# dwkim606/optimal_conv

Measured on AMD Instinct MI355X. Metric: homomorphic convs/sec (conv_then_pack + BN bias, k x k, batch B, N=2^16), higher is better.
Workload: dtype u64; 1 GPU; conv 3 3; ker_wid=3, batch=256, in_wid=16, logN=16, moduli=ckks.DefaultBootstrapParams[6] Q0,Q1 + P=0x1fffffffffe00001, ciphertexts_per_launch_set=4, contexts_per_gpu=4, chunk_nodes=512

## Files before the change

### optimal_conv_amd/csrc/hc_kernels.h

```cpp
#pragma once
#include "hc_arith.h"

#define HC_TPB 256
#ifndef HC_MIN_WAVES
#define HC_MIN_WAVES 4
#endif
#define HC_ROWS_LDS 4096
#define HC_COLS_LDS 4096

struct __attribute__((aligned(16))) HcTw { u64 w, ws; };

#define HC_SMALL_Q(q) ((q) < (1ull << 31))
template <bool B> struct HcBool { static constexpr bool value = B; };
template <int V> struct HcInt { static constexpr int value = V; };
#define HC_COUNT_DISPATCH(n, body) do { switch (n) { case 1: body(HcInt<1>{}); break; case 2: body(HcInt<2>{}); break; case 3: body(HcInt<3>{}); break; case 4: body(HcInt<4>{}); break; \
    case 5: body(HcInt<5>{}); break; case 6: body(HcInt<6>{}); break; case 7: body(HcInt<7>{}); break; case 8: body(HcInt<8>{}); break; default: break; } } while (0)
#define HC_LD(S32, rowptr, j) ((S32) ? hc_ld32(rowptr, j) : (rowptr)[j])
#define HC_ST(S32, rowptr, j, v) do { if (S32) hc_st32(rowptr, j, v); else (rowptr)[j] = (v); } while (0)
#define HC_ROW_DISPATCH(row32, body) do { if (row32) body(HcBool<true>{}); else body(HcBool<false>{}); } while (0)
__device__ __forceinline__ u64 hc_ld32(const u64 *row, size_t j) { return (u64)reinterpret_cast<const u32 *>(row)[j]; }
__device__ __forceinline__ void hc_st32(u64 *row, size_t j, u64 v) { reinterpret_cast<u32 *>(row)[j] = (u32)v; }
struct __attribute__((packed, aligned(4))) HcU64A4 { u64 v; };
__device__ __forceinline__ u64 hc_ldp(const u64 *row, size_t j, bool row32) {
    return reinterpret_cast<const HcU64A4 *>(reinterpret_cast<const char *>(row) + (j << (row32 ? 2 : 3)))->v & (row32 ? 0xFFFFFFFFull : ~0ull);
// ... 1287 lines not shown
                lds[a0] = hc_submod(hc_addmod(hc_submod(Y0[j], m0, q), g0, q), hc_canon8(e0[kk], Q), q);
            }
        }
        __syncthreads();
#pragma unroll
        for (int j = 0; j < HC_B5_ROWS; j++) {
            const int kk = b + j;
            const u32 srcidx = hc_perm_src((u32)((HC_TILE * 16 + kk) * 256 + t), B.gal);
            const u64 d1 = lds[hc_rows_lds(kk ^ 8, (int)(srcidx & 255))], d0 = lds[hc_rows_lds(kk, (int)(srcidx & 255))];
            o[65536 + kk * 256] = FM == HC_FM_FREE ? hc_reduce64(s1[j] + d1, B.m0.mu, Q) : hc_addmod(s1[j], d1, q);
            o[kk * 256] = FM == HC_FM_FREE ? hc_reduce64(s0[j] + d0, B.m0.mu, Q) : hc_addmod(s0[j], d0, q);
        }
    }
}

#define HC_STPB 256
#define HC_STILES 64
#define HC_S_LDS 1024
__device__ __forceinline__ int hc_s_addr(int line, int x) { return x * 4 + line; }
__device__ __forceinline__ int hc_s_pos(int u, int lo) { return (u & ((1 << lo) - 1)) | ((u >> lo) << (lo + 2)); }
template <bool ROWS, int D> __device__ __forceinline__ HcTw hc_s_tw_fwd(const HcTwTab &T, int x, int gline) {
    if (D >= 16) { constexpr int s = D == 128 ? 0 : D == 64 ? 1 : D == 32 ? 2 : 3; const int slot = (1 << s) - 1 + (x >> (8 - s)); return ROWS ? T.rowsA[gline * 16 + slot] : T.colsA[slot]; }
    constexpr int s = D == 8 ? 0 : D == 4 ? 1 : D == 2 ? 2 : 3; const int slot = (1 << s) - 1 + ((x & 15) >> (4 - s));
    return ROWS ? T.rowsB[gline * 256 + slot * 16 + (x >> 4)] : T.colsB[slot * 16 + (x >> 4)];
}
template <bool ROWS, int D> __device__ __forceinline__ HcTw hc_s_tw_inv(const HcTwTab &T, int x, int gline) {
    if (D <= 8) { constexpr int s = D == 1 ? 0 : D == 2 ? 1 : D == 4 ? 2 : 3; const int slot = (8 >> s) - 1 + ((x & 15) >> (s + 1)); return ROWS ? T.rowsB[gline * 256 + slot * 16 + (x >> 4)] : T.colsB[slot * 16 + (x >> 4)]; }
    constexpr int s = D == 16 ? 0 : D == 32 ? 1 : D == 64 ? 2 : 3; const int slot = (8 >> s) - 1 + (x >> (5 + s));
    return ROWS ? T.rowsA[gline * 16 + slot] : T.colsA[slot];
}
// ... 1495 lines not shown
```

### optimal_conv_amd/csrc/hconv.hip

```cpp
#ifdef HC_EMU
#include "hip_emu.h"
#else
#include <hip/hip_runtime.h>
#endif

#include <math.h>
#include <stdarg.h>
#include <stdio.h>
#include <string.h>

#include <map>
#include <utility>
#include <string>
#include <vector>

#include "../../include/hconv.h"
#include "../../include/hconv_test_hooks.h"
#include "hc_kernels.h"
#include "hc_gomath.h"
#ifndef HC_GX_LV
#define HC_GX_LV 64
#endif
#ifndef HC_GX_PW
#define HC_GX_PW 32
#endif
// ... 62 lines not shown
    HcTwTab32 fwd32 = {nullptr, nullptr, nullptr, nullptr}, inv32 = {nullptr, nullptr, nullptr, nullptr};
    HcTwTab inv_f64;
    std::vector<void *> allocs;
};
struct HcEvk { HcTw *q_rows; HcTw *p_rows; u64 *q_mont; bool row_local; bool row256; };
struct HcSwk { u64 *rows = nullptr; int level = 0, beta = 0; };
struct HcProfRec { std::string name; hipEvent_t a, b; };
struct hc_ctx {
    int device = 0, nq = 0, np = 0;
    hipStream_t stream = nullptr;
    std::vector<HcModHost> mods;
    std::map<u64, HcEvk> evk;
    std::map<u64, HcSwk> swk;
    HcTw *idx_pairs = nullptr;
    u64 *idx_mont = nullptr;
    u64 *ws_cts = nullptr; size_t ws_cts_rows = 0;
    u64 *ws_cts2 = nullptr; size_t ws_cts2_rows = 0;
    HcTw *ws_ctc = nullptr; size_t ws_ctc_cts = 0;
    u64 *ws_tmp = nullptr; size_t ws_tmp_rows = 0;
    HcMod *d_mods = nullptr; HcTw *d_csts = nullptr;
    u64 *d_mono = nullptr;
    struct CacheBlk { size_t n = 0; hipEvent_t ev = nullptr; bool pending = false; };
    std::map<char *, CacheBlk> cache_blk; std::map<size_t, std::vector<void *>> cache_free;
    int async_alloc = 0;
#ifdef HC_EMU
    long small_mm_wgs = 0;
#else
    long small_mm_wgs = 1024;
#endif
    long allocs_live = 0;
// ... 15 lines not shown
    u64 *ws_gather = nullptr; size_t ws_gather_rows = 0;
    long small_levels = 16;
    long peer_access = 1;
    int xcd_rows = 1;
    int pack32 = 1;
    int rot_fuse = 1;
    int small32 = 1;
    unsigned peer_warned = 0;
    unsigned peer_enabled = 0;
    long profile = 0;
    std::vector<HcProfRec> prof;
    std::map<std::string, std::pair<double, long>> prof_acc;
    hipEvent_t t0 = nullptr, t1 = nullptr;
    std::string err;
};
struct hc_ker { u64 *d = nullptr; int max_ob = 0; };

static std::string g_create_err;
static int hc_fail(hc_ctx *c, int code, const char *fmt, ...) {
    char buf[512]; va_list ap; va_start(ap, fmt); vsnprintf(buf, sizeof buf, fmt, ap); va_end(ap);
    if (c) c->err = buf; else g_create_err = buf;
    return code;
}
#define HC_HIP(c, call) do { hipError_t e_ = (call); if (e_ != hipSuccess) return hc_fail(c, HC_ERR_HIP, "%s: %s", #call, hipGetErrorString(e_)); } while (0)
#define HC_ENTER(c) do { if (!(c)) return HC_ERR_ARG; HC_HIP(c, hipSetDevice((c)->device)); } while (0)
static void hc_hoist_drop(hc_ctx *c) { c->hoist_cx = nullptr; }
static void hc_hoist_hold(hc_ctx *c, const void *cx, int level) { c->hoist_cx = cx; c->hoist_level = level; }
static int hc_hoist_need(hc_ctx *c, const char *fn, const void *cx, int level) {
    if (c->hoist_cx == cx && c->hoist_level == level) return HC_OK;
    return hc_fail(c, HC_ERR_STATE, "%s: no decomposition of this polynomial at level %d is held (call hc_keyswitch_decompose first)", fn, level);
}
// ... 580 lines not shown
    A->ctc = c->ws_ctc; A->ker = kers; A->tmp = c->ws_tmp; A->cts = cts; A->i0 = 0; A->norm = norm; A->slot0 = 0; A->slot_step = norm;
    A->cts_stride = cts_stride;
    A->m0 = m0.m; A->m1 = m1.m;
    A->q1inv = h_pair(h_inv(m1.m.q % m0.m.q, m0.m.q), m0.m.q);
    A->h = (m1.m.q - 1) >> 1; A->negh0 = m0.m.q - (A->h % m0.m.q);
    return HC_OK;
}

static int hc_prepare_ctc(hc_ctx *c, const HcPtrs &ct_in, int n, const u64 cst[2]) {
    HC_TRY(hc_ensure_ctc(c, (size_t)n));
    HcCtc K; K.m0 = c->mods[0].m; K.m1 = c->mods[1].m;
    K.c0 = h_pair(cst[0] % K.m0.q, K.m0.q); K.c1 = h_pair(cst[1] % K.m1.q, K.m1.q);
    return hc_launch(c, "ctc", hc_k_ctc_pairs, dim3(64, 4, (unsigned)n), ct_in, c->ws_ctc, K);
}

static int hc_loopA_run_set(hc_ctx *c, const HcPtrs &kers, int n, int i_first, int i_stride, int nch, u64 *cts, size_t cts_stride, bool compact, int gm = 1) {
    long chunk = (c->chunk_nodes < 1 ? 1 : c->chunk_nodes) / n; if (chunk < 1) chunk = 1;
    if (chunk > nch) chunk = nch;
    HC_TRY(hc_ensure_tmp(c, (size_t)n * (size_t)chunk * 2));
    HcLoopA A; HC_TRY(hc_fill_loopA(c, &A, kers, cts, cts_stride, i_stride));
    const HcModHost &m0 = c->mods[0], &m1 = c->mods[1];
    for (int j0 = 0; j0 < nch; j0 += (int)chunk) {
        const int nj = (int)((nch - j0) < chunk ? (nch - j0) : chunk);
        A.i0 = i_first + j0 * i_stride;
        A.slot0 = compact ? j0 : A.i0; A.slot_step = compact ? 1 : i_stride;
        A.njobs = 2 * nj; A.gm = gm;
        const dim3 pair = hc_grid(nj, n), flat = hc_grid(2 * nj * n);
        if (gm > 1) {
            const bool f64 = hc_f64_ok(m1.m.q);
            const HcTwTab &t1 = f64 ? m1.inv_f64 : m1.inv;
            HC_TRY(f64 ? hc_launch(c, "a1g_mulsum_rowsinv", hc_k_a1g<1>, pair, A, t1) : hc_launch(c, "a1g_mulsum_rowsinv", hc_k_a1g<0>, pair, A, t1));
            if (f64) HC_TRY(hc_fm_free(m0.m.q) ? hc_launch(c, "a2_colsinv_lift_colsfwd", hc_k_a2<HC_FM_FREE, 1>, flat, A, t1, m0.fwd) : hc_launch(c, "a2_colsinv_lift_colsfwd", hc_k_a2<HC_FM_ALT, 1>, flat, A, t1, m0.fwd));
            else HC_TRY(hc_fm_free(m0.m.q) ? hc_launch(c, "a2_colsinv_lift_colsfwd", hc_k_a2<HC_FM_FREE, 0>, flat, A, t1, m0.fwd) : hc_launch(c, "a2_colsinv_lift_colsfwd", hc_k_a2<HC_FM_ALT, 0>, flat, A, t1, m0.fwd));
            HC_TRY(HC_LAUNCH_FM(m0.m.q, c, "a3g_rowsfwd_sum_rescale", hc_k_a3g, pair, A, m0.fwd));
            continue;
        }
        if (hc_f64_ok(m1.m.q)) {
            HC_TRY(hc_launch(c, "a1_mul_rowsinv", hc_k_a1p<1>, pair, A, m1.inv_f64));
            HC_TRY(hc_fm_free(m0.m.q) ? hc_launch(c, "a2_colsinv_lift_colsfwd", hc_k_a2<HC_FM_FREE, 1>, flat, A, m1.inv_f64, m0.fwd)
                                      : hc_launch(c, "a2_colsinv_lift_colsfwd", hc_k_a2<HC_FM_ALT, 1>, flat, A, m1.inv_f64, m0.fwd));
// ... 95 lines not shown
    if (!rc) rc = hc_launch(c, "evk_div_p", hc_k_pointwise<HC_PW_MULC>, hc_pw_grid(2 * HC_N), (const u64 *)stageq, (const u64 *)stageq, stageq, (size_t)2 * HC_N, m0.m, pinv);
    if (!rc) rc = hc_launch(c, "make_pairs", hc_k_make_pairs, hc_pw_grid(2 * HC_N), (const u64 *)stageq, e.q_rows, (size_t)2 * HC_N, m0.m.q, 0);
    if (!rc) rc = hc_launch(c, "evk_to_mont", hc_k_pointwise<HC_PW_TO_MONT>, hc_pw_grid(2 * HC_N), (const u64 *)stageq, (const u64 *)stageq, e.q_mont, (size_t)2 * HC_N, m0.m, z);
    if (!rc) rc = hc_launch(c, "evk_from_mont", hc_k_pointwise<HC_PW_FROM_MONT>, hc_pw_grid(2 * HC_N), (const u64 *)stage, (const u64 *)stage, stage, (size_t)2 * HC_N, mp.m, z);
    if (!rc) rc = hc_launch(c, "evk_ninv", hc_k_pointwise<HC_PW_MULC>, hc_pw_grid(2 * HC_N), (const u64 *)stage, (const u64 *)stage, stage, (size_t)2 * HC_N, mp.m, h_pair(mp.m.ninv, mp.m.q));
    if (!rc) rc = hc_launch(c, "make_pairs", hc_k_make_pairs, hc_pw_grid(2 * HC_N), (const u64 *)stage, e.p_rows, (size_t)2 * HC_N, mp.m.q, 1);
    if (hipStreamSynchronize(c->stream) != hipSuccess && !rc) rc = hc_fail(c, HC_ERR_HIP, "hc_evk_load: stream synchronize failed");
    if (rc) return rc;
    S.keep(e.q_rows); S.keep(e.p_rows);
    auto it = c->evk.find(galEl);
    if (it != c->evk.end()) { hcx_free(c, it->second.q_rows); hcx_free(c, it->second.p_rows); }
    c->evk[galEl] = e;
    return HC_OK;
}

extern "C" int hc_idx_load(hc_ctx *c, const uint64_t *idx_host) {
    HC_ENTER(c);
    const HcModHost &m0 = c->mods[0];
    HcScratch S(c);
    u64 *stage = nullptr; HC_HIP(c, S.alloc(&stage, (size_t)HC_LOGN * HC_N * sizeof(u64)));
    if (idx_host) {
        HC_HIP(c, hcx_h2d_async(c, stage, idx_host, (size_t)HC_LOGN * HC_N * sizeof(u64)));
    } else {
        HC_HIP(c, hipMemsetAsync(stage, 0, (size_t)HC_LOGN * HC_N * sizeof(u64), c->stream));
        u64 one = 1;
        for (int i = 0; i < HC_LOGN; i++) HC_HIP(c, hcx_h2d_async(c, stage + (size_t)i * HC_N + ((size_t)1 << i), &one, sizeof one));
        HC_HIP(c, hipStreamSynchronize(c->stream));
        u64 *tmp = nullptr; HC_HIP(c, S.alloc(&tmp, (size_t)HC_LOGN * HC_N * sizeof(u64)));
        HC_TRY(HC_LAUNCH_FM(m0.m.q, c, "cols_fwd", hc_k_cols_fwd, dim3(16, HC_LOGN), (const u64 *)stage, tmp, m0.fwd, m0.m.q));
        HC_TRY(HC_LAUNCH_FM(m0.m.q, c, "rows_fwd_canon", hc_k_rows_fwd_canon, dim3(16, HC_LOGN), (const u64 *)tmp, stage, m0.fwd, m0.m.q, m0.m.mu));
    }
    HcTw *pairs = nullptr; HC_HIP(c, S.alloc(&pairs, (size_t)HC_LOGN * HC_N * (sizeof(HcTw) + sizeof(u64))));
    u64 *mont = reinterpret_cast<u64 *>(pairs + (size_t)HC_LOGN * HC_N);
    HcTw z; z.w = z.ws = 0;
    HC_TRY(hc_launch(c, "idx_pairs", hc_k_make_pairs, hc_pw_grid((size_t)HC_LOGN * HC_N), (const u64 *)stage, pairs, (size_t)HC_LOGN * HC_N, m0.m.q, 0));
    HC_TRY(hc_launch(c, "idx_to_mont", hc_k_pointwise<HC_PW_TO_MONT>, hc_pw_grid((size_t)HC_LOGN * HC_N), (const u64 *)stage, (const u64 *)stage, mont, (size_t)HC_LOGN * HC_N, m0.m, z));
    HC_HIP(c, hipStreamSynchronize(c->stream));
    S.keep(pairs);
    if (c->idx_pairs) HC_HIP(c, hcx_free(c, c->idx_pairs));
    c->idx_pairs = pairs; c->idx_mont = mont;
    return HC_OK;
}

static int hc_ker_from_device(hc_ctx *c, u64 *d, int max_ob, bool take, hc_ker **out) {
    u64 *dst = d;
    int rc = HC_OK;
    if (!take) {
        HC_HIP(c, hcx_malloc(c, (void **)&dst, (size_t)max_ob * 2 * HC_N * sizeof(u64)));
        if (hipMemcpyAsync(dst, d, (size_t)max_ob * 2 * HC_N * sizeof(u64), hipMemcpyDeviceToDevice, c->stream) != hipSuccess) rc = hc_fail(c, HC_ERR_HIP, "hc_ker_load: device copy failed");
    }
    if (!rc && hipStreamSynchronize(c->stream) != hipSuccess) rc = hc_fail(c, HC_ERR_HIP, "hc_ker_load: stream synchronize failed");
    if (rc) { hcx_free(c, dst); return rc; }
    hc_ker *k = new hc_ker(); k->d = dst; k->max_ob = max_ob; *out = k;
    return HC_OK;
}
// ... 58 lines not shown
                              int real_ib, int real_ob, int norm, double scale, int trans, hc_ker **out) {
    HC_ENTER(c);
    return hc_prep_ker_impl(c, trans ? "hc_prep_ker_ex" : "hc_prep_ker", ker_in, ker_len, bn_a, in_wid, ker_wid, real_ib, real_ob, norm, scale, trans, 1, 1, out);
}
extern "C" int hc_prep_ker(hc_ctx *c, const double *ker_in, int ker_len, const double *bn_a, int in_wid, int ker_wid,
                           int real_ib, int real_ob, int norm, double scale, hc_ker **out) {
    return hc_prep_ker_ex(c, ker_in, ker_len, bn_a, in_wid, ker_wid, real_ib, real_ob, norm, scale, 0, out);
}
extern "C" int hc_ker_download(hc_ctx *c, const hc_ker *k, uint64_t *host_out) {
    HC_ENTER(c); if (!k || !host_out) return hc_fail(c, HC_ERR_ARG, "hc_ker_download: null");
    const size_t n = (size_t)k->max_ob * 2 * HC_N;
    HC_HIP(c, hipMemcpyAsync(host_out, k->d, n * sizeof(u64), hipMemcpyDeviceToHost, c->stream));
    HC_HIP(c, hipStreamSynchronize(c->stream));
    return HC_OK;
}
extern "C" void hc_ker_free(hc_ctx *c, hc_ker *k) { if (!k) return; if (c) { hipSetDevice(c->device); hipStreamSynchronize(c->stream); } hcx_free(c, k->d); delete k; }

static int hc_fill_loopB(hc_ctx *c, HcLoopB *B, const u64 *src, u64 *dst, const HcEvk &e, int logStep, int step, int norm, u64 galEl, int chunk) {
    const HcModHost &m0 = c->mods[0], &mp = c->mods[(size_t)c->nq];
    B->src = src; B->dst = dst;
    B->tmpC = c->ws_tmp; B->tmpE = c->ws_tmp + (size_t)chunk * HC_N; B->tmpT = c->ws_tmp + (size_t)chunk * 3 * HC_N;
    B->idx = c->idx_pairs + (size_t)logStep * HC_N;
    B->evkQ = e.q_rows; B->evkP = e.p_rows;
    B->idxM = c->idx_mont + (size_t)logStep * HC_N; B->evkQM = e.q_mont;
    B->n0 = 0; B->step = step; B->norm = norm; B->nodes = 1; B->src_stride = 0; B->dst_stride = 0;
    B->m0 = m0.m; B->mp = mp.m;
    B->pmodq = h_pair(mp.m.q % m0.m.q, m0.m.q);
    B->pinv = h_pair(h_inv(mp.m.q % m0.m.q, m0.m.q), m0.m.q);
    B->mu0 = (u64)((((u128)1) << 64) / m0.m.q);
    {
        const double pf = (double)mp.m.q;
        u64 lo = 0, hi = mp.m.q;
        while (lo < hi) { u64 mid = lo + (hi - lo) / 2; if ((u64)((double)mid / pf) >= 1) hi = mid; else lo = mid + 1; }
        B->vthresh = lo;
    }
    B->gal = (u32)(galEl & 0x1FFFF);
    return HC_OK;
}
static int hc_pack_level(hc_ctx *c, const u64 *src, u64 *dst, size_t sstride, size_t dstride, int n, int step, int logStep, int norm, u64 galEl, const HcPtrs *bias_last, const HcPtrs *outs_last = nullptr) {
    auto it = c->evk.find(galEl);
    if (it == c->evk.end()) return hc_fail(c, HC_ERR_STATE, "pack: no switching key loaded for galEl=%llu (the reference panics in permuteNTT)", (unsigned long long)galEl);
    if (!it->second.row_local) return hc_fail(c, HC_ERR_UNSUPPORTED, "pack: galEl=%llu does not permute inside 4096-coefficient tiles (needs max_cnum <= 4096)", (unsigned long long)galEl);
    if (!c->idx_pairs) HC_TRY(hc_idx_load(c, nullptr));
    const int nodes = (step + norm - 1) / norm;
    long chunkl = (c->chunk_nodes < 1 ? 1 : c->chunk_nodes) / n; if (chunkl < 1) chunkl = 1;
    const int chunk = (int)(chunkl < nodes ? chunkl : nodes);
    HC_TRY(hc_ensure_tmp(c, (size_t)n * chunk * 4));
    HcLoopB B; HC_TRY(hc_fill_loopB(c, &B, src, dst, it->second, logStep, step, norm, galEl, n * chunk));
    B.src_stride = sstride; B.dst_stride = dstride;
    if (it->second.row256) B.tmpT = nullptr;
    HcPtrs nobias; memset(&nobias, 0, sizeof nobias);
    const HcModHost &m0 = c->mods[0], &mp = c->mods[(size_t)c->nq];
    for (int n0 = 0; n0 < nodes; n0 += chunk) {
        const int nn = (nodes - n0) < chunk ? (nodes - n0) : chunk;
        B.n0 = n0; B.nodes = nn;
        const dim3 g1 = hc_grid(n * nn), g2 = hc_grid(2 * n * nn);
        if (c->small_levels > 0 && (long)n * nn <= c->small_levels && it->second.row256) {
            const HcPtrs pb = bias_last ? *bias_last : nobias, po = outs_last ? *outs_last : nobias;
            B.tmpT = nullptr;
            const dim3 s1(HC_STILES, (unsigned)(n * nn)), s2(HC_STILES, (unsigned)(2 * n * nn)), s3(HC_STILES, (unsigned)(n * nn), 2);
            HC_TRY(hc_launch<HC_STPB>(c, "b1_node_rowsinv", hc_k_sb1, s1, B, m0.inv));
            HC_TRY(hc_launch<HC_STPB>(c, "b2_colsinv_colsfwdP", hc_k_sb2, s1, B, m0.inv, mp.fwd));
            HC_TRY(hc_launch<HC_STPB>(c, "b3_rowsfwdP_mac_rowsinvP", hc_k_sb3, s3, B, mp.fwd, mp.inv));
            HC_TRY(hc_launch<HC_STPB>(c, "b4_colsinvP_modup_colsfwd", hc_k_sb4, s2, B, mp.inv, m0.fwd));
            HC_TRY(hc_launch<HC_STPB>(c, "b5_rowsfwd_moddown_perm_add", hc_k_sb5, s2, B, m0.fwd, pb, po));
            continue;
        }
        HC_TRY(hc_launch(c, "b1_node_rowsinv", hc_k_b1, g1, B, m0.inv));
        HC_TRY(HC_LAUNCH_FM(mp.m.q, c, "b2_colsinv_colsfwdP", hc_k_b2, g1, B, m0.inv, mp.fwd));
        HC_TRY(HC_LAUNCH_FM(mp.m.q, c, "b3_rowsfwdP_mac_rowsinvP", hc_k_b3p, g1, B, mp.fwd, mp.inv));
        HC_TRY(HC_LAUNCH_FM(m0.m.q, c, "b4_colsinvP_modup_colsfwd", hc_k_b4, g2, B, mp.inv, m0.fwd));
        const HcPtrs pb = bias_last ? *bias_last : nobias, po = outs_last ? *outs_last : nobias;
        if (it->second.row256) HC_TRY(HC_LAUNCH_FM(m0.m.q, c, "b5_rowsfwd_moddown_perm_add", hc_k_b5m, g1, B, m0.fwd, pb, po));
        else HC_TRY(HC_LAUNCH_FM(m0.m.q, c, "b5_rowsfwd_moddown_perm_add", hc_k_b5, g2, B, m0.fwd, pb, po));
    }
    return HC_OK;
}
static int hc_pack_run(hc_ctx *c, u64 *cts, size_t cstride, int n, int max_cnum, int real_cnum, const HcPtrs *bias, int stride_log2 = 0, const HcPtrs *outs = nullptr) {
    if (max_cnum < 1 || real_cnum < 1 || max_cnum % real_cnum || (max_cnum & (max_cnum - 1)) || (real_cnum & (real_cnum - 1)))
        return hc_fail(c, HC_ERR_ARG, "pack: max_cnum=%d real_cnum=%d must be powers of two", max_cnum, real_cnum);
    const int norm = max_cnum / real_cnum;
    int step = max_cnum / 2, logStep = 0;
    for (int i = step; i > 1; i /= 2) logStep++;
    if (stride_log2 < 0 || logStep + stride_log2 >= HC_LOGN) return hc_fail(c, HC_ERR_ARG, "pack: stride_log2=%d out of range", stride_log2);
    int j = HC_LOGN - logStep - stride_log2;
    const size_t pong_one = (size_t)(max_cnum / 2 > 0 ? max_cnum / 2 : 1) * 2, pong_rows = pong_one * (size_t)n;
    if (c->ws_cts2_rows < pong_rows) {
        HC_HIP(c, hipStreamSynchronize(c->stream));
        if (c->ws_cts2) HC_HIP(c, hcx_free(c, c->ws_cts2));
        c->ws_cts2 = nullptr; c->ws_cts2_rows = 0;
        HC_HIP(c, hcx_malloc(c, (void **)&c->ws_cts2, pong_rows * HC_N * sizeof(u64)));
        c->ws_cts2_rows = pong_rows;
    }
    u64 *src = cts, *dst = c->ws_cts2;
    size_t sstride = cstride, dstride = pong_one * HC_N;
    bool bias_done = false, out_done = false;
    while (step >= norm && step >= 1) {
        const bool last = (step / 2 < norm) || step == 1;
        HC_TRY(hc_pack_level(c, src, dst, sstride, dstride, n, step, logStep + stride_log2, norm, (1ull << j) + 1, last ? bias : nullptr, last ? outs : nullptr));
        if (last) { bias_done = true; out_done = outs != nullptr; }
        u64 *t = src; src = dst; dst = t;
        size_t ts = sstride; sstride = dstride; dstride = ts;
        step /= 2; logStep--; j++;
    }
    if (out_done) return HC_OK;
    if (src != cts) for (int z = 0; z < n; z++)
        HC_TRY(hc_copy_d2d(c, cts + (size_t)z * cstride, src + (size_t)z * sstride, 2 * HC_N * sizeof(u64)));
    if (bias && !bias_done) {
        HcTw z0; z0.w = z0.ws = 0;
        for (int z = 0; z < n; z++) if (bias->p[z])
            HC_TRY(hc_launch(c, "bias_add", hc_k_pointwise<HC_PW_ADD>, hc_pw_grid(HC_N), (const u64 *)(cts + (size_t)z * cstride), bias->p[z], cts + (size_t)z * cstride, (size_t)HC_N, c->mods[0].m, z0));
    }
    if (outs) for (int z = 0; z < n; z++) HC_TRY(hc_copy_d2d(c, (void *)outs->p[z], cts + (size_t)z * cstride, 2 * HC_N * sizeof(u64)));
    return HC_OK;
// ... 458 lines not shown
    double sc = prod * smul; int drops = 0, level = 1;
    while (level - drops > 0 && sc / (double)c->mods[(size_t)(level - drops)].m.q >= tgt / 2) { sc /= (double)c->mods[(size_t)(level - drops)].m.q; drops++; }
    if (drops != 1) return hc_fail(c, HC_ERR_STATE, "conv: SetScale would drop %d limbs instead of 1 (scales ct=%g ker=%g out=%g)", drops, ct_scale, ker_scale, out_scale);
    *target = tgt;
    return HC_OK;
}
extern "C" int hc_conv_mult_phase(hc_ctx *c, const uint64_t *ct_in, double ct_scale, const hc_ker *ker, double ker_scale,
                                  int max_ob, int norm, double out_scale, uint64_t *cts_out) {
    HC_ENTER(c);
    if (!ct_in || !ker || !cts_out || ker->max_ob < max_ob) return hc_fail(c, HC_ERR_ARG, "hc_conv_mult_phase: bad arguments");
    u64 cst[2]; double target;
    HC_TRY(hc_loopA_consts(c, ct_scale, ker_scale, max_ob, norm, out_scale, cst, &target));
    HC_TRY(hc_prepare_ctc(c, hc_ptrs1((const u64 *)ct_in), 1, cst));
    return hc_loopA_run(c, ker->d, max_ob, norm, (u64 *)cts_out);
}
static int hc_conv_batch_run(hc_ctx *c, int n, const HcPtrs &ct_in, const HcPtrs &kers, const HcPtrs &bias, bool any_bias, u64 *const *ct_out,
                             int max_ob, int norm, const u64 cst[2], int gm = 1) {
    const int G = n / gm;
    HC_TRY(hc_prepare_ctc(c, ct_in, n, cst));
    HC_TRY(hc_ensure_cts(c, (size_t)G * max_ob * 2));
    const size_t cstride = (size_t)max_ob * 2 * HC_N;
    HC_TRY(hc_loopA_run_set(c, kers, G, 0, norm, max_ob / norm, c->ws_cts, cstride, false, gm));
    HcPtrs outs; memset(&outs, 0, sizeof outs); for (int z = 0; z < G; z++) outs.p[z] = ct_out[z];
    return hc_pack_run(c, c->ws_cts, cstride, G, max_ob, max_ob / norm, any_bias ? &bias : nullptr, 0, &outs);
}
extern "C" int hc_conv_then_pack(hc_ctx *c, const uint64_t *ct_in, double ct_scale, const hc_ker *ker, double ker_scale,
                                 int max_ob, int norm, double out_scale, const uint64_t *bias, uint64_t *ct_out, double *scale_out) {
    HC_ENTER(c);
    if (!ct_in || !ker || !ct_out || ker->max_ob < max_ob) return hc_fail(c, HC_ERR_ARG, "hc_conv_then_pack: bad arguments");
    u64 cst[2]; double target;
    HC_TRY(hc_loopA_consts(c, ct_scale, ker_scale, max_ob, norm, out_scale, cst, &target));
    const double final_scale = target * (double)(max_ob / norm);
    if (final_scale != out_scale) return hc_fail(c, HC_ERR_STATE, "LV or scale after conv then pack, inconsistent");
    u64 *outs[1] = {(u64 *)ct_out};
    HC_TRY(hc_conv_batch_run(c, 1, hc_ptrs1((const u64 *)ct_in), hc_ptrs1(ker->d), hc_ptrs1((const u64 *)bias), bias != nullptr, outs, max_ob, norm, cst));
    if (scale_out) *scale_out = final_scale;
    return HC_OK;
}
extern "C" int hc_conv_then_pack_batch(hc_ctx *c, int n, const uint64_t *const *ct_in, double ct_scale, const hc_ker *const *ker, double ker_scale,
                                       int max_ob, int norm, double out_scale, const uint64_t *const *bias, uint64_t *const *ct_out, double *scale_out) {
    HC_ENTER(c);
    if (n < 1 || n > HC_MAXB) return hc_fail(c, HC_ERR_ARG, "hc_conv_then_pack_batch: n=%d outside 1..%d", n, HC_MAXB);
    if (!ct_in || !ker || !ct_out) return hc_fail(c, HC_ERR_ARG, "hc_conv_then_pack_batch: null");
    HcPtrs pin, pker, pbias; memset(&pin, 0, sizeof pin); memset(&pker, 0, sizeof pker); memset(&pbias, 0, sizeof pbias);
    u64 *outs[HC_MAXB]; bool any_bias = false;
    int G = 0, gm = 0;
    for (int z = 0, z0 = 0; z < n; z++) {
        if (!ct_in[z] || !ker[z] || !ct_out[z] || ker[z]->max_ob < max_ob) return hc_fail(c, HC_ERR_ARG, "hc_conv_then_pack_batch: bad arguments for ciphertext %d", z);
        pin.p[z] = (const u64 *)ct_in[z]; pker.p[z] = ker[z]->d;
        const u64 *b = bias ? (const u64 *)bias[z] : nullptr;
        if (z == 0 || ct_out[z] != ct_out[z - 1]) {
            for (int y = 0; y < G; y++) if (outs[y] == (u64 *)ct_out[z]) return hc_fail(c, HC_ERR_ARG, "hc_conv_then_pack_batch: ct_out of member %d repeats a non-adjacent member's (a group's members must be consecutive)", z);
            if (G == 1) gm = z;
            if (G >= 1 && z - z0 != gm) return hc_fail(c, HC_ERR_ARG, "hc_conv_then_pack_batch: groups of unequal size (%d members, then %d)", gm, z - z0);
            z0 = z; outs[G] = (u64 *)ct_out[z];
            if (b) { pbias.p[G] = b; any_bias = true; }
            G++;
        } else if (b && b != pbias.p[G - 1]) return hc_fail(c, HC_ERR_ARG, "hc_conv_then_pack_batch: bias of member %d conflicts with its group's (the first member's entry; the others NULL or the same pointer)", z);
        if (z == n - 1) { if (G == 1) gm = n; else if (n - z0 != gm) return hc_fail(c, HC_ERR_ARG, "hc_conv_then_pack_batch: groups of unequal size (%d members, then %d)", gm, n - z0); }
    }
    u64 cst[2]; double target;
    HC_TRY(hc_loopA_consts(c, ct_scale, ker_scale, max_ob, norm, out_scale, cst, &target));
    const double final_scale = target * (double)(max_ob / norm);
    if (final_scale != out_scale) return hc_fail(c, HC_ERR_STATE, "LV or scale after conv then pack, inconsistent");
    HC_TRY(hc_conv_batch_run(c, n, pin, pker, pbias, any_bias, outs, max_ob, norm, cst, gm));
    if (scale_out) *scale_out = final_scale;
    return HC_OK;
}

extern "C" int hc_conv_then_pack_sharded(hc_ctx *const *ctxs, int G, const uint64_t *const *ct_in, double ct_scale, const hc_ker *const *ker, double ker_scale,
                                         int max_ob, double out_scale, const uint64_t *bias, uint64_t *ct_out, double *scale_out) {
    if (!ctxs || G < 1 || !ctxs[0]) return HC_ERR_ARG;
    hc_ctx *c0 = ctxs[0];
    HC_ENTER(c0);
    if (G > HC_MAXB || (G & (G - 1)) || !ct_in || !ker || !ct_out) return hc_fail(c0, HC_ERR_ARG, "hc_conv_then_pack_sharded: G=%d must be a power of two <= %d, pointers non-null", G, HC_MAXB);
    if (max_ob < G || max_ob % G) return hc_fail(c0, HC_ERR_ARG, "hc_conv_then_pack_sharded: max_ob=%d must be a multiple of G=%d", max_ob, G);
    int log2g = 0; while ((1 << log2g) < G) log2g++;
    const int nloc = max_ob / G;
    u64 cst[2]; double target;
    HC_TRY(hc_loopA_consts(c0, ct_scale, ker_scale, max_ob, 1, out_scale, cst, &target));
// ... 340 lines not shown
```

Measured before the change: 856.3 conv/s.

## Fold leaf pack-level monomial into cached kernels to skip half the leaf multiplies

```diff
diff --git a/optimal_conv_amd/csrc/hc_kernels.h b/optimal_conv_amd/csrc/hc_kernels.h
--- a/optimal_conv_amd/csrc/hc_kernels.h
+++ b/optimal_conv_amd/csrc/hc_kernels.h
@@ -1325,6 +1325,107 @@
     }
 }
 
+__global__ __launch_bounds__(HC_TPB, HC_W_B1) void hc_k_b1x(HcLoopB B, HcTwTab T0inv) {
+    __shared__ __attribute__((aligned(16))) u64 lds[HC_ROWS_LDS];
+    const int t = threadIdx.x, tid = t & 15, rloc = t >> 4, row = HC_TILE * 16 + rloc;
+    const int job = HC_JOB, z = job / B.nodes, node = job - z * B.nodes, i = (B.n0 + node) * B.norm;
+    const size_t tile = (size_t)HC_TILE * 4096 + t;
+    const u64 *__restrict__ y1 = B.src + (size_t)z * B.src_stride + ((size_t)i * 2 + 1) * 65536 + tile;
+    const u64 *__restrict__ m1 = B.src + (size_t)z * B.src_stride + ((size_t)(i + B.step) * 2 + 1) * 65536 + tile;
+    const HcQ Q = hc_q(B.m0.q);
+    u64 e[16], yy[16];
+#pragma unroll
+    for (int kk = 0; kk < 16; kk++) { e[kk] = m1[kk * 256]; yy[kk] = y1[kk * 256]; }
+#pragma unroll
+    for (int kk = 0; kk < 16; kk++) e[kk] = yy[kk] + Q.q - e[kk];
+    hc_rows_lin_to_lo(lds, t, rloc, tid, e);
+    const HcTw wA = hc_twl_load(T0inv, HC_TILE, t);
+    HC_ROW_SYNC();
+    hc_rows_inv(HcLazy<>{Q}, lds, T0inv, row, rloc, tid, e, &wA);
+    u64 *__restrict__ o = B.tmpC + (size_t)job * 65536 + (size_t)row * 256;
+#pragma unroll
+    for (int hi = 0; hi < 16; hi++) o[hi * 16 + tid] = e[hi];
+}
+template <int FM>
+__device__ __forceinline__ void hc_rows_fwd2_lin_x(u64 (&e0)[16], u64 (&e1)[16], u64 *lds, const HcTwTab &T, const HcTw &wA, int row, int rloc, int tid, int t, const HcQ &Q) {
+    hc_ct_round(HcLazy<FM>{Q}, hc_twl_put(lds, wA, rloc, tid), e0, e1);
+    HC_ROW_SYNC();
+    hc_xchg(lds, [&](int hi) { return hc_rows_lds(rloc, hi * 16 + tid); }, [&](int lo) { return hc_rows_lds(rloc, tid * 16 + lo); }, [] { HC_ROW_SYNC(); }, e0, e1);
+    hc_ct_round(HcLazy<FM>{Q}, HcTwB<false, HcTw>{T.rowsB + row * 256 + tid}, e0, e1);
+    HC_ROW_SYNC();
+    hc_xchg(lds, [&](int lo) { return hc_rows_lds(rloc, tid * 16 + lo); }, [&](int kk) { return hc_rows_lds(kk, t); }, [] { __syncthreads(); }, e0, e1);
+}
+template <int FM>
+__global__ __launch_bounds__(HC_TPB, HC_B5M_WAVES) void hc_k_b5x(HcLoopB B, HcTwTab T0fwd, HcPtrs biases, HcPtrs outs) {
+    __shared__ __attribute__((aligned(16))) u64 lds[HC_ROWS_LDS];
+    const int t = threadIdx.x, tid = t & 15, rloc = t >> 4, row = HC_TILE * 16 + rloc;
+    const int zn = HC_JOB, z = zn / B.nodes, node = zn - z * B.nodes, i = (B.n0 + node) * B.norm;
+    const HcQ Q = hc_q(B.m0.q);
+    const u64 q = Q.q, qinv = B.m0.qinv;
+    const size_t tile = (size_t)HC_TILE * 4096 + t;
+    const u64 *__restrict__ ys = B.src + (size_t)z * B.src_stride + (size_t)i * 2 * 65536 + tile;
+    const u64 *__restrict__ ms = B.src + (size_t)z * B.src_stride + (size_t)(i + B.step) * 2 * 65536 + tile;
+    const u64 *__restrict__ evk = B.evkQM + tile;
+    u64 *__restrict__ o = (outs.p[z] != nullptr ? const_cast<u64 *>(outs.p[z]) : B.dst + (size_t)z * B.dst_stride + (size_t)i * 2 * 65536) + tile;
+    const u64 *__restrict__ bias = biases.p[z] != nullptr ? biases.p[z] + tile : nullptr;
+    const HcTw wA = hc_twl_load(T0fwd, HC_TILE, t);
+    u64 e0[16], e1[16];
+    {
+        const u64 *__restrict__ in = B.tmpE + (size_t)zn * 2 * 65536 + (size_t)row * 256;
+#pragma unroll
+        for (int hi = 0; hi < 16; hi++) { e0[hi] = in[hi * 16 + tid]; e1[hi] = in[65536 + hi * 16 + tid]; }
+    }
+    hc_rows_fwd2_lin_x<FM>(e0, e1, lds, T0fwd, wA, row, rloc, tid, t, Q);
+    __syncthreads();
+#pragma unroll
+    for (int b = 0; b < 16; b += HC_B5_ROWS) {
+        u64 Y0[HC_B5_ROWS], M0[HC_B5_ROWS], Y1[HC_B5_ROWS], M1[HC_B5_ROWS], K0[HC_B5_ROWS], K1[HC_B5_ROWS], bs[HC_B5_ROWS], s0[HC_B5_ROWS], s1[HC_B5_ROWS];
+#pragma unroll
+        for (int j = 0; j < HC_B5_ROWS; j++) {
+            const int off = (b + j) * 256;
+            Y1[j] = ys[65536 + off]; M1[j] = ms[65536 + off]; Y0[j] = ys[off]; M0[j] = ms[off]; K0[j] = evk[off]; K1[j] = evk[65536 + off];
+            bs[j] = bias != nullptr ? bias[off] : 0;
+        }
+#pragma unroll
+        for (int j = 0; j < HC_B5_ROWS; j++) {
+            const int kk = b + j, a0 = hc_rows_lds(kk, t), a1 = hc_rows_lds(kk ^ 8, t);
+            const u64 T = Y1[j] + q - M1[j];
+            u64 g1 = hc_mont_lazy(T, K1[j], q, qinv), g0 = hc_mont_lazy(T, K0[j], q, qinv);
+            if (FM == HC_FM_FREE) {
+                s1[j] = Y1[j] + M1[j]; s0[j] = Y0[j] + M0[j] + bs[j];
+                lds[a1] = g1 + HC_FREE_OFF * q - e1[kk];
+                lds[a0] = Y0[j] + q - M0[j] + g0 + HC_FREE_OFF * q - e0[kk];
+            } else {
+                g1 = hc_canon4(g1, Q); g0 = hc_canon4(g0, Q);
+                s1[j] = hc_addmod(Y1[j], M1[j], q); s0[j] = hc_addmod(hc_addmod(Y0[j], M0[j], q), bs[j], q);
+                lds[a1] = hc_submod(g1, hc_canon8(e1[kk], Q), q);
+                lds[a0] = hc_submod(hc_addmod(hc_submod(Y0[j], M0[j], q), g0, q), hc_canon8(e0[kk], Q), q);
+            }
+        }
+        __syncthreads();
+#pragma unroll
+        for (int j = 0; j < HC_B5_ROWS; j++) {
+            const int kk = b + j;
+            const u32 srcidx = hc_perm_src((u32)((HC_TILE * 16 + kk) * 256 + t), B.gal);
+            const u64 d1 = lds[hc_rows_lds(kk ^ 8, (int)(srcidx & 255))], d0 = lds[hc_rows_lds(kk, (int)(srcidx & 255))];
+            o[65536 + kk * 256] = FM == HC_FM_FREE ? hc_reduce64(s1[j] + d1, B.m0.mu, Q) : hc_addmod(s1[j], d1, q);
+            o[kk * 256] = FM == HC_FM_FREE ? hc_reduce64(s0[j] + d0, B.m0.mu, Q) : hc_addmod(s0[j], d0, q);
+        }
+    }
+}
+__global__ __launch_bounds__(HC_TPB) void hc_k_ker_fold(const u64 *ker, const u64 *mono, u64 *fold, int i0, int norm, int nch, HcMod m0, HcMod m1) {
+    const size_t n = (size_t)nch * 2 * 65536;
+    for (size_t id = (size_t)blockIdx.x * HC_TPB + threadIdx.x; id < n; id += (size_t)gridDim.x * HC_TPB) {
+        const size_t x = id & 65535, r = id >> 16; const int l = (int)(r & 1); const size_t j = r >> 1;
+        const HcMod m = l ? m1 : m0;
+        const u64 k = ker[(((size_t)i0 + j * (size_t)norm) * 2 + l) * 65536 + x];
+        fold[id] = hc_mont(k, hc_mont(mono[(size_t)l * 65536 + x], m.r2, m.q, m.qinv), m.q, m.qinv);
+    }
+}
+__global__ __launch_bounds__(HC_TPB) void hc_k_words_differ(const u64 *a, const u64 *b, size_t n, u32 *differs) {
+    for (size_t i = (size_t)blockIdx.x * HC_TPB + threadIdx.x; i < n; i += (size_t)gridDim.x * HC_TPB) if (a[i] != b[i]) *differs = 1;
+}
+
 #define HC_STPB 256
 #define HC_STILES 64
 #define HC_S_LDS 1024
diff --git a/optimal_conv_amd/csrc/hconv.hip b/optimal_conv_amd/csrc/hconv.hip
--- a/optimal_conv_amd/csrc/hconv.hip
+++ b/optimal_conv_amd/csrc/hconv.hip
@@ -9,6 +9,7 @@
 #include <stdio.h>
 #include <string.h>
 
+#include <atomic>
 #include <map>
 #include <utility>
 #include <string>
@@ -101,6 +102,8 @@
     std::map<u64, HcSwk> swk;
     HcTw *idx_pairs = nullptr;
     u64 *idx_mont = nullptr;
+    bool idx_mono = false;
+    u64 idx_gen = 0;
     u64 *ws_cts = nullptr; size_t ws_cts_rows = 0;
     u64 *ws_cts2 = nullptr; size_t ws_cts2_rows = 0;
     HcTw *ws_ctc = nullptr; size_t ws_ctc_cts = 0;
@@ -146,7 +149,7 @@
     hipEvent_t t0 = nullptr, t1 = nullptr;
     std::string err;
 };
-struct hc_ker { u64 *d = nullptr; int max_ob = 0; };
+struct hc_ker { u64 *d = nullptr; int max_ob = 0; mutable u64 *fold = nullptr; mutable int fold_ob = 0, fold_norm = 0; mutable u64 fold_gen = 0; };
 
 static std::string g_create_err;
 static int hc_fail(hc_ctx *c, int code, const char *fmt, ...) {
@@ -757,16 +760,16 @@
     return hc_launch(c, "ctc", hc_k_ctc_pairs, dim3(64, 4, (unsigned)n), ct_in, c->ws_ctc, K);
 }
 
-static int hc_loopA_run_set(hc_ctx *c, const HcPtrs &kers, int n, int i_first, int i_stride, int nch, u64 *cts, size_t cts_stride, bool compact, int gm = 1) {
+static int hc_loopA_run_set(hc_ctx *c, const HcPtrs &kers, int n, int i_first, int i_stride, int nch, u64 *cts, size_t cts_stride, bool compact, int gm = 1, bool folded = false) {
     long chunk = (c->chunk_nodes < 1 ? 1 : c->chunk_nodes) / n; if (chunk < 1) chunk = 1;
     if (chunk > nch) chunk = nch;
     HC_TRY(hc_ensure_tmp(c, (size_t)n * (size_t)chunk * 2));
-    HcLoopA A; HC_TRY(hc_fill_loopA(c, &A, kers, cts, cts_stride, i_stride));
+    HcLoopA A; HC_TRY(hc_fill_loopA(c, &A, kers, cts, cts_stride, folded ? 1 : i_stride));
     const HcModHost &m0 = c->mods[0], &m1 = c->mods[1];
     for (int j0 = 0; j0 < nch; j0 += (int)chunk) {
         const int nj = (int)((nch - j0) < chunk ? (nch - j0) : chunk);
-        A.i0 = i_first + j0 * i_stride;
-        A.slot0 = compact ? j0 : A.i0; A.slot_step = compact ? 1 : i_stride;
+        A.i0 = folded ? j0 : i_first + j0 * i_stride;
+        A.slot0 = compact ? j0 : i_first + j0 * i_stride; A.slot_step = compact ? 1 : i_stride;
         A.njobs = 2 * nj; A.gm = gm;
         const dim3 pair = hc_grid(nj, n), flat = hc_grid(2 * nj * n);
         if (gm > 1) {
@@ -892,22 +895,33 @@
     return HC_OK;
 }
 
+static int hc_monomial_rows(hc_ctx *c, const HcModHost &m, int s0, int rows, u64 *out, u64 *tmp) {
+    HC_HIP(c, hipMemsetAsync(out, 0, (size_t)rows * HC_N * sizeof(u64), c->stream));
+    u64 one = 1;
+    for (int i = 0; i < rows; i++) HC_HIP(c, hcx_h2d_async(c, out + (size_t)i * HC_N + ((size_t)1 << (s0 + i)), &one, sizeof one));
+    HC_HIP(c, hipStreamSynchronize(c->stream));
+    HC_TRY(HC_LAUNCH_FM(m.m.q, c, "cols_fwd", hc_k_cols_fwd, dim3(16, (unsigned)rows), (const u64 *)out, tmp, m.fwd, m.m.q));
+    return HC_LAUNCH_FM(m.m.q, c, "rows_fwd_canon", hc_k_rows_fwd_canon, dim3(16, (unsigned)rows), (const u64 *)tmp, out, m.fwd, m.m.q, m.m.mu);
+}
+static std::atomic<u64> g_idx_gen{0};
 extern "C" int hc_idx_load(hc_ctx *c, const uint64_t *idx_host) {
     HC_ENTER(c);
     const HcModHost &m0 = c->mods[0];
     HcScratch S(c);
     u64 *stage = nullptr; HC_HIP(c, S.alloc(&stage, (size_t)HC_LOGN * HC_N * sizeof(u64)));
+    u64 *tmp = nullptr; HC_HIP(c, S.alloc(&tmp, (size_t)HC_LOGN * HC_N * sizeof(u64)));
+    bool mono = true;
     if (idx_host) {
+        u64 *der = nullptr; u32 *differs = nullptr, h = 0;
+        HC_HIP(c, S.alloc(&der, (size_t)HC_LOGN * HC_N * sizeof(u64))); HC_HIP(c, S.alloc(&differs, sizeof(u32)));
+        HC_TRY(hc_monomial_rows(c, m0, 0, HC_LOGN, der, tmp));
         HC_HIP(c, hcx_h2d_async(c, stage, idx_host, (size_t)HC_LOGN * HC_N * sizeof(u64)));
-    } else {
-        HC_HIP(c, hipMemsetAsync(stage, 0, (size_t)HC_LOGN * HC_N * sizeof(u64), c->stream));
-        u64 one = 1;
-        for (int i = 0; i < HC_LOGN; i++) HC_HIP(c, hcx_h2d_async(c, stage + (size_t)i * HC_N + ((size_t)1 << i), &one, sizeof one));
+        HC_HIP(c, hipMemsetAsync(differs, 0, sizeof(u32), c->stream));
+        HC_TRY(hc_launch(c, "idx_compare", hc_k_words_differ, hc_pw_grid((size_t)HC_LOGN * HC_N), (const u64 *)stage, (const u64 *)der, (size_t)HC_LOGN * HC_N, differs));
+        HC_HIP(c, hipMemcpyAsync(&h, differs, sizeof h, hipMemcpyDeviceToHost, c->stream));
         HC_HIP(c, hipStreamSynchronize(c->stream));
-        u64 *tmp = nullptr; HC_HIP(c, S.alloc(&tmp, (size_t)HC_LOGN * HC_N * sizeof(u64)));
-        HC_TRY(HC_LAUNCH_FM(m0.m.q, c, "cols_fwd", hc_k_cols_fwd, dim3(16, HC_LOGN), (const u64 *)stage, tmp, m0.fwd, m0.m.q));
-        HC_TRY(HC_LAUNCH_FM(m0.m.q, c, "rows_fwd_canon", hc_k_rows_fwd_canon, dim3(16, HC_LOGN), (const u64 *)tmp, stage, m0.fwd, m0.m.q, m0.m.mu));
-    }
+        mono = h == 0;
+    } else HC_TRY(hc_monomial_rows(c, m0, 0, HC_LOGN, stage, tmp));
     HcTw *pairs = nullptr; HC_HIP(c, S.alloc(&pairs, (size_t)HC_LOGN * HC_N * (sizeof(HcTw) + sizeof(u64))));
     u64 *mont = reinterpret_cast<u64 *>(pairs + (size_t)HC_LOGN * HC_N);
     HcTw z; z.w = z.ws = 0;
@@ -917,6 +931,7 @@
     S.keep(pairs);
     if (c->idx_pairs) HC_HIP(c, hcx_free(c, c->idx_pairs));
     c->idx_pairs = pairs; c->idx_mont = mont;
+    c->idx_mono = mono; c->idx_gen = ++g_idx_gen;
     return HC_OK;
 }
 
@@ -1005,7 +1020,7 @@
     HC_HIP(c, hipStreamSynchronize(c->stream));
     return HC_OK;
 }
-extern "C" void hc_ker_free(hc_ctx *c, hc_ker *k) { if (!k) return; if (c) { hipSetDevice(c->device); hipStreamSynchronize(c->stream); } hcx_free(c, k->d); delete k; }
+extern "C" void hc_ker_free(hc_ctx *c, hc_ker *k) { if (!k) return; if (c) { hipSetDevice(c->device); hipStreamSynchronize(c->stream); } hcx_free(c, k->d); hcx_free(c, k->fold); delete k; }
 
 static int hc_fill_loopB(hc_ctx *c, HcLoopB *B, const u64 *src, u64 *dst, const HcEvk &e, int logStep, int step, int norm, u64 galEl, int chunk) {
     const HcModHost &m0 = c->mods[0], &mp = c->mods[(size_t)c->nq];
@@ -1028,7 +1043,7 @@
     B->gal = (u32)(galEl & 0x1FFFF);
     return HC_OK;
 }
-static int hc_pack_level(hc_ctx *c, const u64 *src, u64 *dst, size_t sstride, size_t dstride, int n, int step, int logStep, int norm, u64 galEl, const HcPtrs *bias_last, const HcPtrs *outs_last = nullptr) {
+static int hc_pack_level(hc_ctx *c, const u64 *src, u64 *dst, size_t sstride, size_t dstride, int n, int step, int logStep, int norm, u64 galEl, const HcPtrs *bias_last, const HcPtrs *outs_last = nullptr, bool folded = false) {
     auto it = c->evk.find(galEl);
     if (it == c->evk.end()) return hc_fail(c, HC_ERR_STATE, "pack: no switching key loaded for galEl=%llu (the reference panics in permuteNTT)", (unsigned long long)galEl);
     if (!it->second.row_local) return hc_fail(c, HC_ERR_UNSUPPORTED, "pack: galEl=%llu does not permute inside 4096-coefficient tiles (needs max_cnum <= 4096)", (unsigned long long)galEl);
@@ -1046,7 +1061,7 @@
         const int nn = (nodes - n0) < chunk ? (nodes - n0) : chunk;
         B.n0 = n0; B.nodes = nn;
         const dim3 g1 = hc_grid(n * nn), g2 = hc_grid(2 * n * nn);
-        if (c->small_levels > 0 && (long)n * nn <= c->small_levels && it->second.row256) {
+        if (!folded && c->small_levels > 0 && (long)n * nn <= c->small_levels && it->second.row256) {
             const HcPtrs pb = bias_last ? *bias_last : nobias, po = outs_last ? *outs_last : nobias;
             B.tmpT = nullptr;
             const dim3 s1(HC_STILES, (unsigned)(n * nn)), s2(HC_STILES, (unsigned)(2 * n * nn)), s3(HC_STILES, (unsigned)(n * nn), 2);
@@ -1057,17 +1072,19 @@
             HC_TRY(hc_launch<HC_STPB>(c, "b5_rowsfwd_moddown_perm_add", hc_k_sb5, s2, B, m0.fwd, pb, po));
             continue;
         }
-        HC_TRY(hc_launch(c, "b1_node_rowsinv", hc_k_b1, g1, B, m0.inv));
+        if (folded) HC_TRY(hc_launch(c, "b1_node_rowsinv", hc_k_b1x, g1, B, m0.inv));
+        else HC_TRY(hc_launch(c, "b1_node_rowsinv", hc_k_b1, g1, B, m0.inv));
         HC_TRY(HC_LAUNCH_FM(mp.m.q, c, "b2_colsinv_colsfwdP", hc_k_b2, g1, B, m0.inv, mp.fwd));
         HC_TRY(HC_LAUNCH_FM(mp.m.q, c, "b3_rowsfwdP_mac_rowsinvP", hc_k_b3p, g1, B, mp.fwd, mp.inv));
         HC_TRY(HC_LAUNCH_FM(m0.m.q, c, "b4_colsinvP_modup_colsfwd", hc_k_b4, g2, B, mp.inv, m0.fwd));
         const HcPtrs pb = bias_last ? *bias_last : nobias, po = outs_last ? *outs_last : nobias;
-        if (it->second.row256) HC_TRY(HC_LAUNCH_FM(m0.m.q, c, "b5_rowsfwd_moddown_perm_add", hc_k_b5m, g1, B, m0.fwd, pb, po));
+        if (folded) HC_TRY(HC_LAUNCH_FM(m0.m.q, c, "b5_rowsfwd_moddown_perm_add", hc_k_b5x, g1, B, m0.fwd, pb, po));
+        else if (it->second.row256) HC_TRY(HC_LAUNCH_FM(m0.m.q, c, "b5_rowsfwd_moddown_perm_add", hc_k_b5m, g1, B, m0.fwd, pb, po));
         else HC_TRY(HC_LAUNCH_FM(m0.m.q, c, "b5_rowsfwd_moddown_perm_add", hc_k_b5, g2, B, m0.fwd, pb, po));
     }
     return HC_OK;
 }
-static int hc_pack_run(hc_ctx *c, u64 *cts, size_t cstride, int n, int max_cnum, int real_cnum, const HcPtrs *bias, int stride_log2 = 0, const HcPtrs *outs = nullptr) {
+static int hc_pack_run(hc_ctx *c, u64 *cts, size_t cstride, int n, int max_cnum, int real_cnum, const HcPtrs *bias, int stride_log2 = 0, const HcPtrs *outs = nullptr, bool leaf_folded = false) {
     if (max_cnum < 1 || real_cnum < 1 || max_cnum % real_cnum || (max_cnum & (max_cnum - 1)) || (real_cnum & (real_cnum - 1)))
         return hc_fail(c, HC_ERR_ARG, "pack: max_cnum=%d real_cnum=%d must be powers of two", max_cnum, real_cnum);
     const int norm = max_cnum / real_cnum;
@@ -1088,7 +1105,8 @@
     bool bias_done = false, out_done = false;
     while (step >= norm && step >= 1) {
         const bool last = (step / 2 < norm) || step == 1;
-        HC_TRY(hc_pack_level(c, src, dst, sstride, dstride, n, step, logStep + stride_log2, norm, (1ull << j) + 1, last ? bias : nullptr, last ? outs : nullptr));
+        HC_TRY(hc_pack_level(c, src, dst, sstride, dstride, n, step, logStep + stride_log2, norm, (1ull << j) + 1, last ? bias : nullptr, last ? outs : nullptr, leaf_folded));
+        leaf_folded = false;
         if (last) { bias_done = true; out_done = outs != nullptr; }
         u64 *t = src; src = dst; dst = t;
         size_t ts = sstride; sstride = dstride; dstride = ts;
@@ -1577,15 +1595,54 @@
     HC_TRY(hc_prepare_ctc(c, hc_ptrs1((const u64 *)ct_in), 1, cst));
     return hc_loopA_run(c, ker->d, max_ob, norm, (u64 *)cts_out);
 }
-static int hc_conv_batch_run(hc_ctx *c, int n, const HcPtrs &ct_in, const HcPtrs &kers, const HcPtrs &bias, bool any_bias, u64 *const *ct_out,
+static int hc_ker_fold(hc_ctx *c, const hc_ker *k, int max_ob, int norm, int s, const u64 **out) {
+    *out = nullptr;
+    if (k->fold && k->fold_ob == max_ob && k->fold_norm == norm && k->fold_gen == c->idx_gen) { *out = k->fold; return HC_OK; }
+    if (k->fold) { HC_HIP(c, hcx_free(c, k->fold)); k->fold = nullptr; }
+    const int nch = (max_ob / 2) / norm;
+    HcScratch S(c);
+    u64 *f = nullptr, *mono = nullptr, *tmp = nullptr;
+    if (S.alloc(&f, (size_t)nch * 2 * HC_N * sizeof(u64)) != hipSuccess || S.alloc(&mono, (size_t)2 * HC_N * sizeof(u64)) != hipSuccess || S.alloc(&tmp, (size_t)HC_N * sizeof(u64)) != hipSuccess) {
+        (void)hipGetLastError();
+        return HC_OK;
+    }
+    for (int l = 0; l < 2; l++) HC_TRY(hc_monomial_rows(c, c->mods[(size_t)l], s, 1, mono + (size_t)l * HC_N, tmp));
+    HC_TRY(hc_launch(c, "ker_fold_monomial", hc_k_ker_fold, hc_pw_grid((size_t)nch * 2 * HC_N), (const u64 *)k->d, (const u64 *)mono, f, max_ob / 2, norm, nch, c->mods[0].m, c->mods[1].m));
+    S.keep(f);
+    k->fold = f; k->fold_ob = max_ob; k->fold_norm = norm; k->fold_gen = c->idx_gen;
+    *out = f;
+    return HC_OK;
+}
+static int hc_conv_fold_leaf(hc_ctx *c, int n, int G, const hc_ker *const *handles, int max_ob, int norm, HcPtrs *folded, bool *use) {
+    *use = false;
+    const int step = max_ob / 2;
+    if (step < 1 || step < norm || (max_ob & (max_ob - 1)) || (norm & (norm - 1))) return HC_OK;
+    int s = 0; for (int i = step; i > 1; i /= 2) s++;
+    if (!c->idx_pairs) HC_TRY(hc_idx_load(c, nullptr));
+    if (!c->idx_mono) return HC_OK;
+    const auto it = c->evk.find((1ull << (HC_LOGN - s)) + 1);
+    if (it == c->evk.end() || !it->second.row256) return HC_OK;
+    if (c->small_levels > 0 && (long)G * (step / norm) <= c->small_levels) return HC_OK;
+    memset(folded, 0, sizeof *folded);
+    for (int z = 0; z < n; z++) { HC_TRY(hc_ker_fold(c, handles[z], max_ob, norm, s, &folded->p[z])); if (!folded->p[z]) return HC_OK; }
+    *use = true;
+    return HC_OK;
+}
+static int hc_conv_batch_run(hc_ctx *c, int n, const HcPtrs &ct_in, const hc_ker *const *handles, const HcPtrs &bias, bool any_bias, u64 *const *ct_out,
                              int max_ob, int norm, const u64 cst[2], int gm = 1) {
     const int G = n / gm;
+    HcPtrs kers, folded; memset(&kers, 0, sizeof kers); for (int z = 0; z < n; z++) kers.p[z] = handles[z]->d;
+    bool fold; HC_TRY(hc_conv_fold_leaf(c, n, G, handles, max_ob, norm, &folded, &fold));
     HC_TRY(hc_prepare_ctc(c, ct_in, n, cst));
     HC_TRY(hc_ensure_cts(c, (size_t)G * max_ob * 2));
     const size_t cstride = (size_t)max_ob * 2 * HC_N;
-    HC_TRY(hc_loopA_run_set(c, kers, G, 0, norm, max_ob / norm, c->ws_cts, cstride, false, gm));
+    if (fold) {
+        const int half = (max_ob / 2) / norm;
+        HC_TRY(hc_loopA_run_set(c, kers, G, 0, norm, half, c->ws_cts, cstride, false, gm));
+        HC_TRY(hc_loopA_run_set(c, folded, G, max_ob / 2, norm, half, c->ws_cts, cstride, false, gm, true));
+    } else HC_TRY(hc_loopA_run_set(c, kers, G, 0, norm, max_ob / norm, c->ws_cts, cstride, false, gm));
     HcPtrs outs; memset(&outs, 0, sizeof outs); for (int z = 0; z < G; z++) outs.p[z] = ct_out[z];
-    return hc_pack_run(c, c->ws_cts, cstride, G, max_ob, max_ob / norm, any_bias ? &bias : nullptr, 0, &outs);
+    return hc_pack_run(c, c->ws_cts, cstride, G, max_ob, max_ob / norm, any_bias ? &bias : nullptr, 0, &outs, fold);
 }
 extern "C" int hc_conv_then_pack(hc_ctx *c, const uint64_t *ct_in, double ct_scale, const hc_ker *ker, double ker_scale,
                                  int max_ob, int norm, double out_scale, const uint64_t *bias, uint64_t *ct_out, double *scale_out) {
@@ -1596,7 +1653,7 @@
     const double final_scale = target * (double)(max_ob / norm);
     if (final_scale != out_scale) return hc_fail(c, HC_ERR_STATE, "LV or scale after conv then pack, inconsistent");
     u64 *outs[1] = {(u64 *)ct_out};
-    HC_TRY(hc_conv_batch_run(c, 1, hc_ptrs1((const u64 *)ct_in), hc_ptrs1(ker->d), hc_ptrs1((const u64 *)bias), bias != nullptr, outs, max_ob, norm, cst));
+    HC_TRY(hc_conv_batch_run(c, 1, hc_ptrs1((const u64 *)ct_in), &ker, hc_ptrs1((const u64 *)bias), bias != nullptr, outs, max_ob, norm, cst));
     if (scale_out) *scale_out = final_scale;
     return HC_OK;
 }
@@ -1605,12 +1662,12 @@
     HC_ENTER(c);
     if (n < 1 || n > HC_MAXB) return hc_fail(c, HC_ERR_ARG, "hc_conv_then_pack_batch: n=%d outside 1..%d", n, HC_MAXB);
     if (!ct_in || !ker || !ct_out) return hc_fail(c, HC_ERR_ARG, "hc_conv_then_pack_batch: null");
-    HcPtrs pin, pker, pbias; memset(&pin, 0, sizeof pin); memset(&pker, 0, sizeof pker); memset(&pbias, 0, sizeof pbias);
+    HcPtrs pin, pbias; memset(&pin, 0, sizeof pin); memset(&pbias, 0, sizeof pbias);
     u64 *outs[HC_MAXB]; bool any_bias = false;
     int G = 0, gm = 0;
     for (int z = 0, z0 = 0; z < n; z++) {
         if (!ct_in[z] || !ker[z] || !ct_out[z] || ker[z]->max_ob < max_ob) return hc_fail(c, HC_ERR_ARG, "hc_conv_then_pack_batch: bad arguments for ciphertext %d", z);
-        pin.p[z] = (const u64 *)ct_in[z]; pker.p[z] = ker[z]->d;
+        pin.p[z] = (const u64 *)ct_in[z];
         const u64 *b = bias ? (const u64 *)bias[z] : nullptr;
         if (z == 0 || ct_out[z] != ct_out[z - 1]) {
             for (int y = 0; y < G; y++) if (outs[y] == (u64 *)ct_out[z]) return hc_fail(c, HC_ERR_ARG, "hc_conv_then_pack_batch: ct_out of member %d repeats a non-adjacent member's (a group's members must be consecutive)", z);
@@ -1626,7 +1683,7 @@
     HC_TRY(hc_loopA_consts(c, ct_scale, ker_scale, max_ob, norm, out_scale, cst, &target));
     const double final_scale = target * (double)(max_ob / norm);
     if (final_scale != out_scale) return hc_fail(c, HC_ERR_STATE, "LV or scale after conv then pack, inconsistent");
-    HC_TRY(hc_conv_batch_run(c, n, pin, pker, pbias, any_bias, outs, max_ob, norm, cst, gm));
+    HC_TRY(hc_conv_batch_run(c, n, pin, ker, pbias, any_bias, outs, max_ob, norm, cst, gm));
     if (scale_out) *scale_out = final_scale;
     return HC_OK;
 }
```

Result: faster. 865.6 conv/s, median of 6 (+1.1%).
